# hku-mars/GS-SDF

Measured on NVIDIA H100. Metric: train_steps_per_s, higher is better.
Workload: dtype f32

## Files before the change

gs-sdf_b200/csrc/raster.cu:

```cuda
#include "common.cuh"
#include "conic.cuh"

namespace gssdf {

constexpr int kRasterThreads = 256;
constexpr int kRasterWarps = kRasterThreads / 32;
constexpr int kBatch = 128;
constexpr float kNearN = 0.05f, kFarN = 100.f;
constexpr float kAlphaThreshold = 1.f / 255.f;
constexpr int kRecF4 = 4;
constexpr int kRecBytes = kRecF4 * 16;

__global__ void __launch_bounds__(256)
pack_records_kernel(const gssdf_counts *counts, const float *__restrict__ ray_transforms,
                    const float *__restrict__ colors, const float *__restrict__ opacities,
                    const float *__restrict__ normals, float4 *__restrict__ rec, float4 *__restrict__ conic,
                    float *__restrict__ zero_a, int zero_a_stride, float extent) {
    const int nnz = counts->nnz;
    const int i = blockIdx.x * blockDim.x + threadIdx.x;
    if (i >= nnz) return;
    const float *M = ray_transforms + 9 * (int64_t)i;
    const float *c = colors + 3 * (int64_t)i;
    const float *n = normals + 3 * (int64_t)i;
    float4 *r = rec + kRecF4 * (int64_t)i;
    const float opac = opacities[i];
    r[0] = make_float4(M[0], M[1], M[2], M[3]);
    r[1] = make_float4(M[4], M[5], M[6], M[7]);
    r[2] = make_float4(M[8], opac, c[0], c[1]);
    r[3] = make_float4(c[2], n[0], n[1], n[2]);
    float q[6];
    uint32_t rect[2];
    splat_conic(M, opac, extent, q, rect);
    conic[kConicF4 * (int64_t)i] = make_float4(q[0], q[1], q[2], q[3]);
    conic[kConicF4 * (int64_t)i + 1] = make_float4(q[4], q[5], __uint_as_float(rect[0]), __uint_as_float(rect[1]));
    if (zero_a) {
        for (int k = 0; k < zero_a_stride; ++k) zero_a[(int64_t)i * zero_a_stride + k] = 0.f;
    }
}

__global__ void __launch_bounds__(256)
splat_conics_kernel(const gssdf_counts *counts, const float *__restrict__ ray_transforms, const float *__restrict__ opacities,
                    float4 *__restrict__ conic, float extent) {
    const int i = blockIdx.x * blockDim.x + threadIdx.x;
    if (i >= counts->nnz) return;
    float q[6];
    uint32_t rect[2];
    splat_conic(ray_transforms + 9 * (int64_t)i, opacities[i], extent, q, rect);
    conic[kConicF4 * (int64_t)i] = make_float4(q[0], q[1], q[2], q[3]);
    conic[kConicF4 * (int64_t)i + 1] = make_float4(q[4], q[5], __uint_as_float(rect[0]), __uint_as_float(rect[1]));
}

struct TileInfo {
    int cam, tile, rs, re;
    int tx, ty;
};

__device__ __forceinline__ TileInfo tile_info(int C, int tw, int th, const int32_t *offsets, const gssdf_counts *counts) {
    TileInfo t;
    const int n_tiles = tw * th;
    const int bin = blockIdx.x;
    t.cam = bin / n_tiles;
    t.tile = bin % n_tiles;
    t.ty = t.tile / tw;
    t.tx = t.tile % tw;
    const int n_isects = counts->n_isects;
    t.rs = min(offsets[bin], n_isects);
    t.re = (bin == C * n_tiles - 1) ? n_isects : min(offsets[bin + 1], n_isects);
    return t;
}

__device__ __forceinline__ void pixel_of_thread(int &lx, int &ly) {
    const int lane = threadIdx.x & 31, warp = threadIdx.x >> 5;
    lx = (warp & 1) * 8 + (lane & 7);
    ly = (warp >> 1) * 4 + (lane >> 3);
}

struct __align__(16) Stage {
    float4 rec[kBatch * kRecF4];
    int ids[kBatch];
    int meta[kBatch];
    float acc[kRasterWarps][kBatch];
};

__global__ void __launch_bounds__(kRasterThreads)
tile_cull_kernel(int C, int tw, int th, const int32_t *__restrict__ offsets, const gssdf_counts *counts,
                 const int32_t *__restrict__ flatten_ids, const float4 *__restrict__ conic, int2 *__restrict__ clist,
                 int32_t *__restrict__ ccount) {
    __shared__ int s_wc[kRasterThreads / 32];
    const TileInfo ti = tile_info(C, tw, th, offsets, counts);
    const float ox = ti.tx * kTile + 0.5f, oy = ti.ty * kTile + 0.5f;
    const int lane = threadIdx.x & 31, warp = threadIdx.x >> 5;
    int count = 0;
    for (int c0 = ti.rs; c0 < ti.re; c0 += kRasterThreads) {
        const int idx = c0 + threadIdx.x;
        int g = 0;
        unsigned mask = 0u;
        if (idx < ti.re) {
            g = flatten_ids[idx];
            mask = cull_mask(__ldg(conic + kConicF4 * (int64_t)g), __ldg(conic + kConicF4 * (int64_t)g + 1), ox, oy);
        }
        const unsigned bal = __ballot_sync(0xffffffffu, mask != 0u);
        if (lane == 0) s_wc[warp] = __popc(bal);
        __syncthreads();
        int before = 0, total = 0;
#pragma unroll
        for (int w = 0; w < kRasterThreads / 32; ++w) {
            const int c = s_wc[w];
            if (w < warp) before += c;
            total += c;
        }
        if (mask != 0u) clist[ti.rs + count + before + __popc(bal & ((1u << lane) - 1u))] = make_int2(g, ((idx - ti.rs) << 8) | (int)mask);
        count += total;
        __syncthreads();
    }
    if (threadIdx.x == 0) ccount[blockIdx.x] = count;
}

__device__ __forceinline__ void issue_batch(Stage &st, uint64_t *bar, const float4 *__restrict__ rec,
                                            const int2 *__restrict__ clist, int start, int n) {
    const int t = threadIdx.x;
    if (t < n) {
        const int2 e = clist[start + t];
        st.ids[t] = e.x;
        st.meta[t] = e.y;
#pragma unroll
        for (int w = 0; w < kRasterWarps; ++w) st.acc[w][t] = 0.f;
        bulk_g2s(&st.rec[t * kRecF4], rec + kRecF4 * (int64_t)e.x, kRecBytes, bar);
        mbar_arrive_expect_tx(bar, kRecBytes);
    } else {
        mbar_arrive(bar);
    }
}

template <bool DISTORT>
__global__ void __launch_bounds__(kRasterThreads)
raster2dgs_fwd_kernel(const gssdf_raster2dgs_fwd_args a, const float4 *__restrict__ rec, const int2 *__restrict__ clist,
                      const int32_t *__restrict__ ccount, int tw, int th) {
    extern __shared__ __align__(16) unsigned char s_raw_fwd[];
    Stage *s_stage = reinterpret_cast<Stage *>(s_raw_fwd);
    __shared__ __align__(8) uint64_t s_bar[2];
    const TileInfo ti = tile_info(a.C, tw, th, a.offsets, a.counts);
    const int W = a.image_width, H = a.image_height;
    int lx, ly;
    pixel_of_thread(lx, ly);
    const int i = ti.ty * kTile + ly, j = ti.tx * kTile + lx;
    const bool inside = i < H && j < W;
    const float px = (float)j + 0.5f, py = (float)i + 0.5f;
    const int64_t pix = ((int64_t)ti.cam * H + i) * W + j;
    const int lane = threadIdx.x & 31;

    if (threadIdx.x == 0) {
        mbar_init(&s_bar[0], kRasterThreads);
        mbar_init(&s_bar[1], kRasterThreads);
        fence_mbar_init();
    }
    __syncthreads();

    const int n_total = ccount[blockIdx.x];
    const int c_end = ti.rs + n_total;
    const int nb = (n_total + kBatch - 1) / kBatch;
    if (nb > 0) issue_batch(s_stage[0], &s_bar[0], rec, clist, ti.rs, min(kBatch, n_total));
    if (nb > 1) issue_batch(s_stage[1], &s_bar[1], rec, clist, ti.rs + kBatch, min(kBatch, n_total - kBatch));

    float T = 1.f;
    float pc0 = 0.f, pc1 = 0.f, pc2 = 0.f, pn0 = 0.f, pn1 = 0.f, pn2 = 0.f;
    float dout = 0.f, M1 = 0.f, M2 = 0.f, distort = 0.f, median_depth = 0.f;
    int cur_idx = 0, median_idx = 0;
    bool done = !inside;
    int waited = 0;

    for (int b = 0; b < nb; ++b) {
        Stage &st = s_stage[b & 1];
        mbar_wait(&s_bar[b & 1], (b >> 1) & 1);
        waited = b + 1;
        const int start = ti.rs + b * kBatch;
        const int bn = min(kBatch, c_end - start);
        const int warp_id = threadIdx.x >> 5;
        for (int t0 = 0; t0 < bn; t0 += 32) {
          if (__all_sync(0xffffffffu, done)) break;
          const int my_meta = (t0 + lane < bn) ? st.meta[t0 + lane] : 0;
          unsigned todo = __ballot_sync(0xffffffffu, (my_meta >> warp_id) & 1);
          while (todo) {
            const int src = __ffs(todo) - 1;
            const int t = t0 + src;
            todo &= todo - 1;
            if (__all_sync(0xffffffffu, done)) break;
            const int sorted_idx = ti.rs + (__shfl_sync(0xffffffffu, my_meta, src) >> 8);
            const float4 r0 = st.rec[t * kRecF4 + 0], r1 = st.rec[t * kRecF4 + 1], r2 = st.rec[t * kRecF4 + 2], r3 = st.rec[t * kRecF4 + 3];
            const float hux = px * r1.z - r0.x, huy = px * r1.w - r0.y, huz = px * r2.x - r0.z;
            const float hvx = py * r1.z - r0.w, hvy = py * r1.w - r1.x, hvz = py * r2.x - r1.y;
            const float rcx = huy * hvz - huz * hvy, rcy = huz * hvx - hux * hvz, rcz = hux * hvy - huy * hvx;
            bool ok = !done && rcz != 0.f;
            const float inv_rcz = __fdividef(1.f, rcz);
            const float sx = rcx * inv_rcz, sy = rcy * inv_rcz;
            const float sigma = 0.5f * (sx * sx + sy * sy);
            const float depth = sx * r1.z + sy * r1.w + r2.x;
            ok = ok && !(depth < kNearN);
            const float alpha = fminf(0.999f, r2.y * __expf(-sigma));
            ok = ok && !(sigma < 0.f || alpha < kAlphaThreshold);
            const float next_T = T * (1.f - alpha);
            if (ok && next_T <= 1e-4f) { done = true; ok = false; }
            float vis = 0.f;
            if (ok) {
                vis = alpha * T;
                pc0 += r2.z * vis; pc1 += r2.w * vis; pc2 += r3.x * vis;
                dout += depth * vis;
                pn0 += r3.y * vis; pn1 += r3.z * vis; pn2 += r3.w * vis;
                if (DISTORT) {
                    const float A = 1.f - T;
                    const float m = kFarN / (kFarN - kNearN) * (1.f - kNearN / depth);
                    distort += (m * m * A + M1 - 2.f * m * M2) * vis;
                    M1 += m * m * vis;
                    M2 += m * vis;
                }
                if (T > 0.5f) { median_depth = depth; median_idx = sorted_idx; }
                cur_idx = sorted_idx;
                T = next_T;
            }
            if (__any_sync(0xffffffffu, ok)) {
                const float v = warp_sum(vis);
                if (lane == 0) st.acc[warp_id][t] = v;
            }
          }
        }
        const int n_done = __syncthreads_count(done);
        if (threadIdx.x < bn) {
            float v = 0.f;
#pragma unroll
            for (int w = 0; w < kRasterWarps; ++w) v += st.acc[w][threadIdx.x];
            if (v != 0.f) atomicAdd(a.visibilities + st.ids[threadIdx.x], v);
        }
        if (n_done == kRasterThreads) break;
        __syncthreads();
        if (b + 2 < nb) {
            const int s2 = ti.rs + (b + 2) * kBatch;
            issue_batch(st, &s_bar[b & 1], rec, clist, s2, min(kBatch, c_end - s2));
        }
    }
    {
        const int issued = min(nb, waited + 1);
        for (int b = waited; b < issued; ++b) mbar_wait(&s_bar[b & 1], (b >> 1) & 1);
    }

    if (inside) {
        a.render_depths[pix] = dout;
        a.render_alphas[pix] = 1.f - T;
        if (DISTORT) reinterpret_cast<float2 *>(a.render_Ts)[pix] = make_float2(M1, M2);
        float b0 = 0.f, b1 = 0.f, b2 = 0.f;
        if (a.backgrounds) { b0 = a.backgrounds[3 * ti.cam]; b1 = a.backgrounds[3 * ti.cam + 1]; b2 = a.backgrounds[3 * ti.cam + 2]; }
        a.render_colors[3 * pix] = pc0 + T * b0;
        a.render_colors[3 * pix + 1] = pc1 + T * b1;
        a.render_colors[3 * pix + 2] = pc2 + T * b2;
        a.render_normals[3 * pix] = pn0;
        a.render_normals[3 * pix + 1] = pn1;
        a.render_normals[3 * pix + 2] = pn2;
        a.last_ids[pix] = cur_idx;
        if (DISTORT) a.render_distort[pix] = distort;
        a.render_median[pix] = median_depth;
        a.median_ids[pix] = median_idx;
    }
}

constexpr int kBwdThreads = 128;
constexpr int kBwdWarps = kBwdThreads / 32;
constexpr int kBwdBatch = 64;
constexpr int kBwdMinBlocks = 5;

template <bool ABS>
struct __align__(16) BwdStageT {
    float4 rec[kBwdBatch * kRecF4];
    float part[kBwdWarps * kBwdBatch * 16];
    float gabs[ABS ? kBwdWarps * 2 * kBwdBatch : 4];
    int ids[kBwdBatch];
    int meta[kBwdBatch];
};

template <bool ABS>
__device__ __forceinline__ void issue_batch_bwd(BwdStageT<ABS> &st, uint64_t *bar, const float4 *__restrict__ rec,
                                                const int2 *__restrict__ clist, int last, int n) {
    const int t = threadIdx.x;
    float4 *part4 = reinterpret_cast<float4 *>(st.part);
#pragma unroll
    for (int k = t; k < kBwdWarps * kBwdBatch * 4; k += kBwdThreads) part4[k] = make_float4(0.f, 0.f, 0.f, 0.f);
    if (ABS) {
#pragma unroll
        for (int k = t; k < kBwdWarps * 2 * kBwdBatch; k += kBwdThreads) st.gabs[k] = 0.f;
    }
    if (t < n) {
        const int2 e = clist[last - t];
        st.ids[t] = e.x;
        st.meta[t] = e.y;
        bulk_g2s(&st.rec[t * kRecF4], rec + kRecF4 * (int64_t)e.x, kRecBytes, bar);
        mbar_arrive_expect_tx(bar, kRecBytes);
    } else {
        mbar_arrive(bar);
    }
}

struct BwdPixel {
    float T;
    float bc0, bc1, bc2, bn0, bn1, bn2, bd;
    float vc0, vc1, vc2, vd, va, vn0, vn1, vn2, v_median;
    int bin_final, median_idx;
};

__device__ __forceinline__ void bwd_pixel_init(BwdPixel &P, const gssdf_raster2dgs_bwd_args &a, const TileInfo &ti, int lx, int ly) {
    const int W = a.image_width, H = a.image_height;
    const int i = ti.ty * kTile + ly, j = ti.tx * kTile + lx;
    const bool inside = i < H && j < W;
    const int64_t pix = inside ? ((int64_t)ti.cam * H + i) * W + j : 0;
    P.T = inside ? 1.f - a.render_alphas[pix] : 1.f;
    P.bc0 = P.bc1 = P.bc2 = P.bn0 = P.bn1 = P.bn2 = P.bd = 0.f;
    P.bin_final = inside ? a.last_ids[pix] : -1;
    P.median_idx = inside ? a.median_ids[pix] : -1;
    P.vc0 = P.vc1 = P.vc2 = P.vd = P.va = P.vn0 = P.vn1 = P.vn2 = P.v_median = 0.f;
    if (inside) {
        P.vc0 = a.v_render_colors[3 * pix]; P.vc1 = a.v_render_colors[3 * pix + 1]; P.vc2 = a.v_render_colors[3 * pix + 2];
        P.vd = a.v_render_depths[pix];
        P.va = a.v_render_alphas[pix];
        P.vn0 = a.v_render_normals[3 * pix]; P.vn1 = a.v_render_normals[3 * pix + 1]; P.vn2 = a.v_render_normals[3 * pix + 2];
        P.v_median = a.v_render_median[pix];
    }
    if (a.backgrounds)
        P.va -= a.backgrounds[3 * ti.cam] * P.vc0 + a.backgrounds[3 * ti.cam + 1] * P.vc1 + a.backgrounds[3 * ti.cam + 2] * P.vc2;
    P.va *= P.T;
}

__device__ __forceinline__ bool bwd_pixel_splat(BwdPixel &P, float px, float py, int idx, const float4 r0, const float4 r1, const float4 r2,
                                                const float4 r3, float g[16]) {
    const float hux = px * r1.z - r0.x, huy = px * r1.w - r0.y, huz = px * r2.x - r0.z;
    const float hvx = py * r1.z - r0.w, hvy = py * r1.w - r1.x, hvz = py * r2.x - r1.y;
    const float rcx = huy * hvz - huz * hvy, rcy = huz * hvx - hux * hvz, rcz = hux * hvy - huy * hvx;
    bool valid = idx <= P.bin_final && rcz != 0.f;
    const float inv_rcz = __fdividef(1.f, rcz);
    const float sx = rcx * inv_rcz, sy = rcy * inv_rcz;
    const float sigma = 0.5f * (sx * sx + sy * sy);
    const float depth = sx * r1.z + sy * r1.w + r2.x;
    valid = valid && !(depth < kNearN);
    const float opac = r2.y;
    const float vis = __expf(-sigma);
    const float alpha = fminf(0.999f, opac * vis);
    valid = valid && !(sigma < 0.f || alpha < kAlphaThreshold);
    if (valid) {
        float v_depth = (idx == P.median_idx) ? P.v_median : 0.f;
        const float ra = __fdividef(1.f, 1.f - alpha);
        P.T *= ra;
        const float T = P.T;
        const float fac = alpha * T;
        g[0] += fac * P.vc0; g[1] += fac * P.vc1; g[2] += fac * P.vc2;
        g[3] += fac * P.vn0; g[4] += fac * P.vn1; g[5] += fac * P.vn2;
        float v_alpha = (r2.z * T - P.bc0 * ra) * P.vc0 + (r2.w * T - P.bc1 * ra) * P.vc1 + (r3.x * T - P.bc2 * ra) * P.vc2;
        v_alpha += (r3.y * T - P.bn0 * ra) * P.vn0 + (r3.z * T - P.bn1 * ra) * P.vn1 + (r3.w * T - P.bn2 * ra) * P.vn2;
        v_alpha += ra * P.va;
        v_alpha += (depth * T - P.bd * ra) * P.vd;
        if (opac * vis <= 0.999f) {
            v_depth += fac * P.vd;
            const float v_G = opac * v_alpha;
            const float vsx = v_G * -vis * sx + v_depth * r1.z;
            const float vsy = v_G * -vis * sy + v_depth * r1.w;
            const float vsxz = vsx * inv_rcz, vsyz = vsy * inv_rcz;
            const float vrx = vsxz, vry = vsyz, vrz = -(vsxz * sx + vsyz * sy);
            const float vhux = hvy * vrz - hvz * vry, vhuy = hvz * vrx - hvx * vrz, vhuz = hvx * vry - hvy * vrx;
            const float vhvx = vry * huz - vrz * huy, vhvy = vrz * hux - vrx * huz, vhvz = vrx * huy - vry * hux;
            g[6] -= vhux; g[7] -= vhuy; g[8] -= vhuz;
            g[9] -= vhvx; g[10] -= vhvy; g[11] -= vhvz;
            g[12] += px * vhux + py * vhvx + v_depth * sx;
            g[13] += px * vhuy + py * vhvy + v_depth * sy;
            g[14] += px * vhuz + py * vhvz + v_depth;
            g[15] += vis * v_alpha;
        }
        P.bc0 += r2.z * fac; P.bc1 += r2.w * fac; P.bc2 += r3.x * fac;
        P.bd += depth * fac;
        P.bn0 += r3.y * fac; P.bn1 += r3.z * fac; P.bn2 += r3.w * fac;
    }
    return valid;
}

template <bool ABS>
__global__ void __launch_bounds__(kBwdThreads, kBwdMinBlocks)
raster2dgs_bwd_kernel(const gssdf_raster2dgs_bwd_args a, const float4 *__restrict__ rec, const int2 *__restrict__ clist,
                      const int32_t *__restrict__ ccount, float *__restrict__ vrec, int tw, int th) {
    using BwdStage = BwdStageT<ABS>;
    extern __shared__ __align__(16) unsigned char s_raw[];
    BwdStage *s_stage = reinterpret_cast<BwdStage *>(s_raw);
    __shared__ __align__(8) uint64_t s_bar[2];
    const TileInfo ti = tile_info(a.C, tw, th, a.offsets, a.counts);
    const int n_total = ccount[blockIdx.x];
    if (n_total <= 0) return;
    const int c_last = ti.rs + n_total - 1;
    const int lane = threadIdx.x & 31, warp = threadIdx.x >> 5;
    const int wb = (warp & 1) + 4 * (warp >> 1);
    const int lx = (warp & 1) * 8 + (lane & 7), ly = (warp >> 1) * 8 + (lane >> 3);
    const float px = (float)(ti.tx * kTile + lx) + 0.5f, py = (float)(ti.ty * kTile + ly) + 0.5f;

    if (threadIdx.x == 0) {
        mbar_init(&s_bar[0], kBwdThreads);
        mbar_init(&s_bar[1], kBwdThreads);
        fence_mbar_init();
    }
    __syncthreads();

    BwdPixel P0, P1;
    bwd_pixel_init(P0, a, ti, lx, ly);
    bwd_pixel_init(P1, a, ti, lx, ly + 4);
    const int warp_bin_final = warp_max_i(max(P0.bin_final, P1.bin_final));

    const int nb = (n_total + kBwdBatch - 1) / kBwdBatch;
    issue_batch_bwd(s_stage[0], &s_bar[0], rec, clist, c_last, min(kBwdBatch, n_total));
    if (nb > 1) issue_batch_bwd(s_stage[1], &s_bar[1], rec, clist, c_last - kBwdBatch, min(kBwdBatch, n_total - kBwdBatch));

    for (int b = 0; b < nb; ++b) {
        BwdStage &st = s_stage[b & 1];
        mbar_wait(&s_bar[b & 1], (b >> 1) & 1);
        const int last = c_last - b * kBwdBatch;
        const int bn = min(kBwdBatch, last - ti.rs + 1);
        float *part = st.part + warp * kBwdBatch * 16;
        for (int t0 = 0; t0 < bn; t0 += 32) {
          const int my_meta = (t0 + lane < bn) ? st.meta[t0 + lane] : 0;
          unsigned todo = __ballot_sync(0xffffffffu, ((my_meta >> wb) & 5) && (ti.rs + (my_meta >> 8) <= warp_bin_final));
          while (todo) {
            const int src = __ffs(todo) - 1;
            const int t = t0 + src;
            todo &= todo - 1;
            const int m = __shfl_sync(0xffffffffu, my_meta, src);
            const int idx = ti.rs + (m >> 8);
            const float4 r0 = st.rec[t * kRecF4 + 0], r1 = st.rec[t * kRecF4 + 1], r2 = st.rec[t * kRecF4 + 2], r3 = st.rec[t * kRecF4 + 3];
            float g[16];
#pragma unroll
            for (int k = 0; k < 16; ++k) g[k] = 0.f;
            bool any = false;
            if ((m >> wb) & 1) any = bwd_pixel_splat(P0, px, py, idx, r0, r1, r2, r3, g);
            if ((m >> (wb + 2)) & 1) any |= bwd_pixel_splat(P1, px, py + 4.f, idx, r0, r1, r2, r3, g);
            if (!__any_sync(0xffffffffu, any)) continue;

            float h8[8], h4[4], h2[2], h1;
            const bool b4 = lane & 16, b3 = lane & 8, b2 = lane & 4, b1 = lane & 2;
#pragma unroll
            for (int k = 0; k < 8; ++k) {
                const float send = b4 ? g[k] : g[k + 8], keep = b4 ? g[k + 8] : g[k];
                h8[k] = keep + __shfl_xor_sync(0xffffffffu, send, 16);
            }
#pragma unroll
            for (int k = 0; k < 4; ++k) {
                const float send = b3 ? h8[k] : h8[k + 4], keep = b3 ? h8[k + 4] : h8[k];
                h4[k] = keep + __shfl_xor_sync(0xffffffffu, send, 8);
            }
#pragma unroll
            for (int k = 0; k < 2; ++k) {
                const float send = b2 ? h4[k] : h4[k + 2], keep = b2 ? h4[k + 2] : h4[k];
                h2[k] = keep + __shfl_xor_sync(0xffffffffu, send, 4);
            }
            {
                const float send = b1 ? h2[0] : h2[1], keep = b1 ? h2[1] : h2[0];
                h1 = keep + __shfl_xor_sync(0xffffffffu, send, 2);
            }
            h1 += __shfl_xor_sync(0xffffffffu, h1, 1);
            const int comp = lane >> 1;
            if ((lane & 1) == 0) part[t * 16 + comp] = h1;
            if (ABS) {
                if (lane == 16) st.gabs[(2 * warp) * kBwdBatch + t] = fabsf(h1 * r2.x);
                if (lane == 22) st.gabs[(2 * warp + 1) * kBwdBatch + t] = fabsf(h1 * r2.x);
            }
          }
        }
        __syncthreads();
        const float4 *part4 = reinterpret_cast<const float4 *>(st.part);
        for (int e = threadIdx.x; e < bn * 4; e += kBwdThreads) {
            float4 v = part4[e];
#pragma unroll
            for (int w = 1; w < kBwdWarps; ++w) {
                const float4 p = part4[w * kBwdBatch * 4 + e];
                v.x += p.x; v.y += p.y; v.z += p.z; v.w += p.w;
            }
            if (v.x != 0.f || v.y != 0.f || v.z != 0.f || v.w != 0.f)
                atomicAdd(reinterpret_cast<float4 *>(vrec) + 4 * (int64_t)st.ids[e >> 2] + (e & 3), v);
        }
        if (ABS) {
            for (int e = threadIdx.x; e < bn * 2; e += kBwdThreads) {
                const int t = e >> 1, k = e & 1;
                float v = 0.f;
#pragma unroll
                for (int w = 0; w < kBwdWarps; ++w) v += st.gabs[(2 * w + k) * kBwdBatch + t];
                if (v != 0.f) atomicAdd(a.v_means2d_abs + 2 * (int64_t)st.ids[t] + k, v);
            }
        }
        __syncthreads();
        if (b + 2 < nb) {
            const int l2 = c_last - (b + 2) * kBwdBatch;
            issue_batch_bwd(st, &s_bar[b & 1], rec, clist, l2, min(kBwdBatch, l2 - ti.rs + 1));
        }
    }
}

__global__ void __launch_bounds__(256)
raster_bwd_finalize_kernel(const gssdf_raster2dgs_bwd_args a, const float4 *__restrict__ vrec) {
    const int nnz = a.counts->nnz;
    const int i = blockIdx.x * blockDim.x + threadIdx.x;
    if (i >= nnz) return;
    const float4 g0 = vrec[4 * (int64_t)i], g1 = vrec[4 * (int64_t)i + 1], g2 = vrec[4 * (int64_t)i + 2], g3 = vrec[4 * (int64_t)i + 3];
    float *vc = a.v_colors + 3 * (int64_t)i;
    vc[0] = g0.x; vc[1] = g0.y; vc[2] = g0.z;
    float *vn = a.v_normals + 3 * (int64_t)i;
    vn[0] = g0.w; vn[1] = g1.x; vn[2] = g1.y;
    float *vm = a.v_ray_transforms + 9 * (int64_t)i;
    vm[0] = g1.z; vm[1] = g1.w; vm[2] = g2.x;
    vm[3] = g2.y; vm[4] = g2.z; vm[5] = g2.w;
    vm[6] = g3.x; vm[7] = g3.y; vm[8] = g3.z;
    a.v_opacities[i] = g3.w;
    if (a.v_means2d) { a.v_means2d[2 * (int64_t)i] = 0.f; a.v_means2d[2 * (int64_t)i + 1] = 0.f; }
    if (a.v_densify) {
        const float mz = a.ray_transforms[9 * (int64_t)i + 8];
        a.v_densify[2 * (int64_t)i] = g2.x * mz;
        a.v_densify[2 * (int64_t)i + 1] = g2.w * mz;
    }
}

__device__ __forceinline__ void cam_rot(const float *viewmats, int cam, float R[9]) {
    const float *v = viewmats + 16 * cam;
#pragma unroll
    for (int r = 0; r < 3; ++r)
#pragma unroll
        for (int c = 0; c < 3; ++c) R[r * 3 + c] = v[r * 4 + c];
}

__global__ void __launch_bounds__(256) render_post_fwd_kernel(const gssdf_render_post_fwd_args a) {
    const int64_t P = (int64_t)a.image_width * a.image_height;
    const int64_t p = (int64_t)blockIdx.x * blockDim.x + threadIdx.x;
    if (p >= P * a.C) return;
    const int cam = (int)(p / P);
    float R[9];
    cam_rot(a.viewmats, cam, R);
    const float al = a.render_alphas[p], d = a.render_depths[p];
    float ed = d / al;
    if (isnan(ed)) ed = 0.f;
    else if (isinf(ed)) ed = ed > 0 ? 3.402823466e38f : -3.402823466e38f;
    reinterpret_cast<float4 *>(a.out_colors)[p] =
        make_float4(a.render_colors[3 * p], a.render_colors[3 * p + 1], a.render_colors[3 * p + 2], ed);
    const float n0 = a.render_normals[3 * p], n1 = a.render_normals[3 * p + 1], n2 = a.render_normals[3 * p + 2];
#pragma unroll
    for (int c = 0; c < 3; ++c) a.out_normals[3 * p + c] = n0 * R[c] + n1 * R[3 + c] + n2 * R[6 + c];
}

__global__ void __launch_bounds__(256) render_post_bwd_kernel(const gssdf_render_post_bwd_args a) {
    const int64_t P = (int64_t)a.image_width * a.image_height;
    const int64_t p = (int64_t)blockIdx.x * blockDim.x + threadIdx.x;
    if (p >= P * a.C) return;
    const int cam = (int)(p / P);
    float R[9];
    cam_rot(a.viewmats, cam, R);
    const float4 vo = reinterpret_cast<const float4 *>(a.v_out_colors)[p];
    a.v_render_colors[3 * p] = vo.x; a.v_render_colors[3 * p + 1] = vo.y; a.v_render_colors[3 * p + 2] = vo.z;
    const float al = a.render_alphas[p], d = a.render_depths[p];
    const float ed = d / al;
    float vdep = 0.f, val = a.v_alphas_in ? a.v_alphas_in[p] : 0.f;
    if (!(isnan(ed) || isinf(ed))) {
        vdep = vo.w / al;
        val += -vo.w * d / (al * al);
    }
    a.v_render_depths[p] = vdep;
    a.v_render_alphas[p] = val;
    const float g0 = a.v_out_normals[3 * p], g1 = a.v_out_normals[3 * p + 1], g2 = a.v_out_normals[3 * p + 2];
#pragma unroll
    for (int r = 0; r < 3; ++r) a.v_render_normals[3 * p + r] = g0 * R[r * 3] + g1 * R[r * 3 + 1] + g2 * R[r * 3 + 2];
}

__global__ void __launch_bounds__(256) l1_loss_kernel(const gssdf_l1_loss_args a, int64_t n_pix) {
    const int64_t p = (int64_t)blockIdx.x * blockDim.x + threadIdx.x;
    float part = 0.f;
    if (p < n_pix) {
        const float4 o = reinterpret_cast<const float4 *>(a.out_colors)[p];
        const float4 g = reinterpret_cast<const float4 *>(a.gt)[p];
        const float sr = a.w_rgb / (3.f * (float)n_pix), sd = a.w_depth / (float)n_pix;
        const float d0 = o.x - g.x, d1 = o.y - g.y, d2 = o.z - g.z, d3 = o.w - g.w;
        part = sr * (fabsf(d0) + fabsf(d1) + fabsf(d2)) + sd * fabsf(d3);
        auto sgn = [](float x) { return x > 0.f ? 1.f : (x < 0.f ? -1.f : 0.f); };
        reinterpret_cast<float4 *>(a.v_out_colors)[p] = make_float4(sr * sgn(d0), sr * sgn(d1), sr * sgn(d2), sd * sgn(d3));
    }
    part = warp_sum(part);
    __shared__ float s_part[8];
    if ((threadIdx.x & 31) == 0) s_part[threadIdx.x >> 5] = part;
    __syncthreads();
    if (threadIdx.x == 0) {
        float s = 0.f;
        for (int w = 0; w < 8; ++w) s += s_part[w];
        atomicAdd(a.loss_out, s);
    }
}

}

using namespace gssdf;

extern "C" int gssdf_l1_loss(const gssdf_l1_loss_args *a, gssdf_stream_t stream) {
    GSSDF_REQUIRE(a != nullptr, GSSDF_EINVAL, "l1_loss: null args");
    GSSDF_REQUIRE(a->C > 0 && a->image_width > 0 && a->image_height > 0, GSSDF_EINVAL, "l1_loss: bad image size");
    GSSDF_REQUIRE(a->out_colors && a->gt && a->loss_out && a->v_out_colors, GSSDF_EINVAL, "l1_loss: null pointer");
    const int64_t n = (int64_t)a->C * a->image_width * a->image_height;
    l1_loss_kernel<<<cdiv(n, 256), 256, 0, (cudaStream_t)stream>>>(*a, n);
    GSSDF_LAUNCH_OK("l1_loss_kernel");
    return GSSDF_OK;
}

struct RasterWs {
    float4 *rec;
    float4 *conic;
    int2 *clist;
    int32_t *ccount;
    float4 *vrec;
    size_t fwd_bytes, bwd_bytes;
};

static RasterWs carve_ws(void *base, int C, int W, int H, int cap, int64_t isect_cap) {
    const size_t n = (size_t)(cap > 0 ? cap : 1), I = (size_t)(isect_cap > 0 ? isect_cap : 1);
    const size_t tiles = (size_t)(C > 0 ? C : 1) * cdiv(W > 0 ? W : 1, kTile) * cdiv(H > 0 ? H : 1, kTile);
    char *p = reinterpret_cast<char *>(base);
    RasterWs w;
    size_t off = 0;
    w.rec = reinterpret_cast<float4 *>(p + off); off += align_up(n * kRecBytes, 256);
    w.conic = reinterpret_cast<float4 *>(p + off); off += align_up(n * kConicF4 * 16, 256);
    w.clist = reinterpret_cast<int2 *>(p + off); off += align_up(I * sizeof(int2), 256);
    w.ccount = reinterpret_cast<int32_t *>(p + off); off += align_up(tiles * sizeof(int32_t), 256);
    w.fwd_bytes = off;
    w.vrec = reinterpret_cast<float4 *>(p + off); off += align_up(n * 64, 256);
    w.bwd_bytes = off;
    return w;
}

extern "C" size_t gssdf_raster2dgs_workspace_bytes(int32_t C, int32_t W, int32_t H, int32_t cap, int64_t isect_cap) {
    return carve_ws(nullptr, C, W, H, cap, isect_cap).fwd_bytes;
}
extern "C" size_t gssdf_raster2dgs_bwd_workspace_bytes(int32_t C, int32_t W, int32_t H, int32_t cap, int64_t isect_cap) {
    return carve_ws(nullptr, C, W, H, cap, isect_cap).bwd_bytes;
}

static int check_raster_common(const char *who, int C, int W, int H, int tile_size, int channels) {
    GSSDF_REQUIRE(C > 0 && W > 0 && H > 0, GSSDF_EINVAL, "%s: C, width, height must be positive", who);
    GSSDF_REQUIRE(tile_size == kTile, GSSDF_EUNSUPPORTED, "%s: tile_size %d unsupported (GS-SDF renders with 16)", who, tile_size);
    GSSDF_REQUIRE(channels == 3, channels <= 0 || channels > 512 ? GSSDF_EINVAL : GSSDF_EUNSUPPORTED,
                  "%s: Unsupported number of color channels: %d", who, channels);
    return GSSDF_OK;
}

extern "C" int gssdf_splat_conics(const gssdf_splat_conics_args *a, gssdf_stream_t stream) {
    GSSDF_REQUIRE(a != nullptr, GSSDF_EINVAL, "splat_conics: null args");
    GSSDF_REQUIRE(a->cap >= 0 && a->image_width > 0 && a->image_height > 0, GSSDF_EINVAL, "splat_conics: bad sizes");
    if (a->cap == 0) return GSSDF_OK;
    GSSDF_REQUIRE(a->counts && a->ray_transforms && a->opacities && a->conics, GSSDF_EINVAL, "splat_conics: null pointer");
    GSSDF_REQUIRE(((uintptr_t)a->conics & 15) == 0, GSSDF_EINVAL, "splat_conics: conics must be 16-byte aligned");
    splat_conics_kernel<<<cdiv(a->cap, 256), 256, 0, (cudaStream_t)stream>>>(a->counts, a->ray_transforms, a->opacities,
                                                                            reinterpret_cast<float4 *>(a->conics),
                                                                            (float)max(a->image_width, a->image_height));
    GSSDF_LAUNCH_OK("splat_conics_kernel");
    return GSSDF_OK;
}

static int pack_and_cull(const char *who, const RasterWs &w, const gssdf_counts *counts, int C, int W, int H, int cap,
                         const float *ray_transforms, const float *colors, const float *opacities, const float *normals,
                         const int32_t *offsets, const int32_t *flatten_ids, float *zero_a, int zero_stride, cudaStream_t st) {
    const int tw = cdiv(W, kTile), th = cdiv(H, kTile);
    if (cap > 0) {
        pack_records_kernel<<<cdiv(cap, 256), 256, 0, st>>>(counts, ray_transforms, colors, opacities, normals, w.rec, w.conic, zero_a,
                                                           zero_stride, (float)max(W, H));
        GSSDF_LAUNCH_OK("pack_records_kernel");
    }
    tile_cull_kernel<<<C * tw * th, kRasterThreads, 0, st>>>(C, tw, th, offsets, counts, flatten_ids, w.conic, w.clist, w.ccount);
    GSSDF_LAUNCH_OK("tile_cull_kernel");
    (void)who;
    return GSSDF_OK;
}

extern "C" int gssdf_raster2dgs_fwd(const gssdf_raster2dgs_fwd_args *a, gssdf_stream_t stream) {
    GSSDF_REQUIRE(a != nullptr, GSSDF_EINVAL, "raster2dgs_fwd: null args");
    int rc = check_raster_common("raster2dgs_fwd", a->C, a->image_width, a->image_height, a->tile_size, a->channels);
    if (rc) return rc;
    GSSDF_REQUIRE(a->counts && a->offsets && a->render_colors && a->render_depths && a->render_alphas && a->render_normals &&
                      a->render_median && a->last_ids && a->median_ids && (a->render_distort != nullptr) == (a->render_Ts != nullptr),
                  GSSDF_EINVAL, "raster2dgs_fwd: null output / counts / offsets");
    GSSDF_REQUIRE(a->cap == 0 || (a->ray_transforms && a->colors && a->opacities && a->normals && a->flatten_ids && a->visibilities),
                  GSSDF_EINVAL, "raster2dgs_fwd: null splat input");
    GSSDF_REQUIRE(a->isect_cap >= 0, GSSDF_EINVAL, "raster2dgs_fwd: negative isect_cap");
    GSSDF_REQUIRE(a->workspace && a->workspace_bytes >= gssdf_raster2dgs_workspace_bytes(a->C, a->image_width, a->image_height, a->cap,
                                                                                         a->isect_cap),
                  GSSDF_ENOMEM, "raster2dgs_fwd: workspace too small");
    cudaStream_t st = (cudaStream_t)stream;
    const int tw = cdiv(a->image_width, kTile), th = cdiv(a->image_height, kTile);
    const RasterWs w = carve_ws(a->workspace, a->C, a->image_width, a->image_height, a->cap, a->isect_cap);
    rc = pack_and_cull("raster2dgs_fwd", w, a->counts, a->C, a->image_width, a->image_height, a->cap, a->ray_transforms, a->colors,
                       a->opacities, a->normals, a->offsets, a->flatten_ids, a->visibilities, 1, st);
    if (rc) return rc;
    GSSDF_CUDA_OK(cudaFuncSetAttribute(raster2dgs_fwd_kernel<true>, cudaFuncAttributeMaxDynamicSharedMemorySize, (int)(2 * sizeof(Stage))));
    GSSDF_CUDA_OK(cudaFuncSetAttribute(raster2dgs_fwd_kernel<false>, cudaFuncAttributeMaxDynamicSharedMemorySize, (int)(2 * sizeof(Stage))));
    if (a->prof_start) GSSDF_CUDA_OK(cudaEventRecord((cudaEvent_t)a->prof_start, st));
    if (a->render_distort)
        raster2dgs_fwd_kernel<true><<<a->C * tw * th, kRasterThreads, 2 * sizeof(Stage), st>>>(*a, w.rec, w.clist, w.ccount, tw, th);
    else
        raster2dgs_fwd_kernel<false><<<a->C * tw * th, kRasterThreads, 2 * sizeof(Stage), st>>>(*a, w.rec, w.clist, w.ccount, tw, th);
    GSSDF_LAUNCH_OK("raster2dgs_fwd_kernel");
    if (a->prof_stop) GSSDF_CUDA_OK(cudaEventRecord((cudaEvent_t)a->prof_stop, st));
    return GSSDF_OK;
}

extern "C" int gssdf_raster2dgs_bwd(const gssdf_raster2dgs_bwd_args *a, gssdf_stream_t stream) {
    GSSDF_REQUIRE(a != nullptr, GSSDF_EINVAL, "raster2dgs_bwd: null args");
    int rc = check_raster_common("raster2dgs_bwd", a->C, a->image_width, a->image_height, a->tile_size, a->channels);
    if (rc) return rc;
    GSSDF_REQUIRE(a->v_render_distort == nullptr, GSSDF_EUNSUPPORTED,
                  "raster2dgs_bwd: distortion-loss cotangent is outside the GS-SDF path (distloss=false)");
    if (a->cap == 0) return GSSDF_OK;
    GSSDF_REQUIRE(a->counts && a->offsets && a->flatten_ids && a->ray_transforms && a->colors && a->opacities && a->normals &&
                      a->render_alphas && a->last_ids && a->median_ids && a->v_render_colors && a->v_render_depths &&
                      a->v_render_alphas && a->v_render_normals && a->v_render_median,
                  GSSDF_EINVAL, "raster2dgs_bwd: null input");
    GSSDF_REQUIRE(a->v_ray_transforms && a->v_colors && a->v_opacities && a->v_normals, GSSDF_EINVAL, "raster2dgs_bwd: null output");
    GSSDF_REQUIRE(a->isect_cap >= 0, GSSDF_EINVAL, "raster2dgs_bwd: negative isect_cap");
    GSSDF_REQUIRE(a->workspace && a->workspace_bytes >= gssdf_raster2dgs_bwd_workspace_bytes(a->C, a->image_width, a->image_height,
                                                                                             a->cap, a->isect_cap),
                  GSSDF_ENOMEM, "raster2dgs_bwd: workspace too small");
    cudaStream_t st = (cudaStream_t)stream;
    const int tw = cdiv(a->image_width, kTile), th = cdiv(a->image_height, kTile);
    const RasterWs w = carve_ws(a->workspace, a->C, a->image_width, a->image_height, a->cap, a->isect_cap);
    if (!a->reuse_fwd) {
        rc = pack_and_cull("raster2dgs_bwd", w, a->counts, a->C, a->image_width, a->image_height, a->cap, a->ray_transforms, a->colors,
                           a->opacities, a->normals, a->offsets, a->flatten_ids, nullptr, 0, st);
        if (rc) return rc;
    }
    GSSDF_CUDA_OK(cudaMemsetAsync(w.vrec, 0, (size_t)a->cap * 64, st));
    if (a->v_means2d_abs) GSSDF_CUDA_OK(cudaMemsetAsync(a->v_means2d_abs, 0, (size_t)a->cap * 2 * sizeof(float), st));
    if (a->prof_start) GSSDF_CUDA_OK(cudaEventRecord((cudaEvent_t)a->prof_start, st));
    auto launch = [&](auto kern, size_t smem) -> int {
        GSSDF_CUDA_OK(cudaFuncSetAttribute(kern, cudaFuncAttributeMaxDynamicSharedMemorySize, (int)smem));
        kern<<<a->C * tw * th, kBwdThreads, smem, st>>>(*a, w.rec, w.clist, w.ccount, reinterpret_cast<float *>(w.vrec), tw, th);
        return GSSDF_OK;
    };
    rc = a->v_means2d_abs ? launch(raster2dgs_bwd_kernel<true>, 2 * sizeof(BwdStageT<true>))
                          : launch(raster2dgs_bwd_kernel<false>, 2 * sizeof(BwdStageT<false>));
    if (rc) return rc;
    GSSDF_LAUNCH_OK("raster2dgs_bwd_kernel");
    if (a->prof_stop) GSSDF_CUDA_OK(cudaEventRecord((cudaEvent_t)a->prof_stop, st));
    raster_bwd_finalize_kernel<<<cdiv(a->cap, 256), 256, 0, st>>>(*a, w.vrec);
    GSSDF_LAUNCH_OK("raster_bwd_finalize_kernel");
    return GSSDF_OK;
}

extern "C" int gssdf_render_post_fwd(const gssdf_render_post_fwd_args *a, gssdf_stream_t stream) {
    GSSDF_REQUIRE(a != nullptr, GSSDF_EINVAL, "render_post_fwd: null args");
    GSSDF_REQUIRE(a->C > 0 && a->image_width > 0 && a->image_height > 0, GSSDF_EINVAL, "render_post_fwd: bad image size");
    GSSDF_REQUIRE(a->viewmats && a->render_colors && a->render_depths && a->render_alphas && a->render_normals && a->out_colors &&
                      a->out_normals,
                  GSSDF_EINVAL, "render_post_fwd: null pointer");
    const int64_t n = (int64_t)a->C * a->image_width * a->image_height;
    render_post_fwd_kernel<<<cdiv(n, 256), 256, 0, (cudaStream_t)stream>>>(*a);
    GSSDF_LAUNCH_OK("render_post_fwd_kernel");
    return GSSDF_OK;
}

extern "C" int gssdf_render_post_bwd(const gssdf_render_post_bwd_args *a, gssdf_stream_t stream) {
    GSSDF_REQUIRE(a != nullptr, GSSDF_EINVAL, "render_post_bwd: null args");
    GSSDF_REQUIRE(a->C > 0 && a->image_width > 0 && a->image_height > 0, GSSDF_EINVAL, "render_post_bwd: bad image size");
    GSSDF_REQUIRE(a->viewmats && a->render_depths && a->render_alphas && a->v_out_colors && a->v_out_normals && a->v_render_colors &&
                      a->v_render_depths && a->v_render_alphas && a->v_render_normals,
                  GSSDF_EINVAL, "render_post_bwd: null pointer");
    const int64_t n = (int64_t)a->C * a->image_width * a->image_height;
    render_post_bwd_kernel<<<cdiv(n, 256), 256, 0, (cudaStream_t)stream>>>(*a);
    GSSDF_LAUNCH_OK("render_post_bwd_kernel");
    return GSSDF_OK;
}
```

Baseline: 192.7.

## Have each forward raster thread shade two pixels with half the threads per tile

The forward rasterizer now launches 128 threads per 16x16 tile, and each thread composites two pixels four rows apart. The shared-memory splat record is loaded once and reused for both pixels, and per-warp ballots skip splats whose cull-mask bits miss both halves. The change also swaps __expf for a direct ex2.approx, sets min-blocks launch bounds, and refreshes warp liveness only when a pixel saturates. The cost is higher register pressure, with two sets of accumulators per thread, plus more divergent branching in the inner loop.

```diff
diff --git a/gs-sdf_b200/csrc/raster.cu b/gs-sdf_b200/csrc/raster.cu
--- a/gs-sdf_b200/csrc/raster.cu
+++ b/gs-sdf_b200/csrc/raster.cu
@@ -4,8 +4,6 @@
 namespace gssdf {
 
 constexpr int kRasterThreads = 256;
-constexpr int kRasterWarps = kRasterThreads / 32;
-constexpr int kBatch = 128;
 constexpr float kNearN = 0.05f, kFarN = 100.f;
 constexpr float kAlphaThreshold = 1.f / 255.f;
 constexpr int kRecF4 = 4;
@@ -69,17 +67,17 @@
     return t;
 }
 
-__device__ __forceinline__ void pixel_of_thread(int &lx, int &ly) {
-    const int lane = threadIdx.x & 31, warp = threadIdx.x >> 5;
-    lx = (warp & 1) * 8 + (lane & 7);
-    ly = (warp >> 1) * 4 + (lane >> 3);
-}
+constexpr int kFwdThreads = 128;
+constexpr int kFwdWarps = kFwdThreads / 32;
+constexpr int kBatch = 128;
+constexpr int kFwdMinBlocks = 8;
+constexpr int kFwdMinBlocksDistort = 6;
 
 struct __align__(16) Stage {
     float4 rec[kBatch * kRecF4];
     int ids[kBatch];
     int meta[kBatch];
-    float acc[kRasterWarps][kBatch];
+    float acc[kFwdWarps][kBatch];
 };
 
 __global__ void __launch_bounds__(kRasterThreads)
@@ -124,7 +122,7 @@
         st.ids[t] = e.x;
         st.meta[t] = e.y;
 #pragma unroll
-        for (int w = 0; w < kRasterWarps; ++w) st.acc[w][t] = 0.f;
+        for (int w = 0; w < kFwdWarps; ++w) st.acc[w][t] = 0.f;
         bulk_g2s(&st.rec[t * kRecF4], rec + kRecF4 * (int64_t)e.x, kRecBytes, bar);
         mbar_arrive_expect_tx(bar, kRecBytes);
     } else {
@@ -132,8 +130,95 @@
     }
 }
 
+static_assert(kBatch <= kFwdThreads, "issue_batch gathers one record per thread");
+
+__device__ __forceinline__ float exp_neg_half(float rho2) {
+    float y;
+    asm("ex2.approx.ftz.f32 %0, %1;" : "=f"(y) : "f"(rho2 * (-0.5f * 1.4426950408889634f)));
+    return y;
+}
+
+struct FwdPixel {
+    float T;
+    float pc0, pc1, pc2, pn0, pn1, pn2, dout, median_depth;
+    float M1, M2, distort;
+    int cur_idx, median_idx;
+    bool done;
+};
+
+struct FwdHit {
+    float alpha, depth;
+    bool ok;
+};
+
+__device__ __forceinline__ FwdHit fwd_pixel_test(const FwdPixel &P, float px, float py, const float4 r0, const float4 r1, const float4 r2) {
+    const float hux = px * r1.z - r0.x, huy = px * r1.w - r0.y, huz = px * r2.x - r0.z;
+    const float hvx = py * r1.z - r0.w, hvy = py * r1.w - r1.x, hvz = py * r2.x - r1.y;
+    const float rcx = huy * hvz - huz * hvy, rcy = huz * hvx - hux * hvz, rcz = hux * hvy - huy * hvx;
+    FwdHit h;
+    h.ok = !P.done && rcz != 0.f;
+    const float inv_rcz = __fdividef(1.f, rcz);
+    const float sx = rcx * inv_rcz, sy = rcy * inv_rcz;
+    const float rho2 = sx * sx + sy * sy;
+    h.depth = sx * r1.z + sy * r1.w + r2.x;
+    h.ok = h.ok && !(h.depth < kNearN);
+    h.alpha = fminf(0.999f, r2.y * exp_neg_half(rho2));
+    h.ok = h.ok && !(h.alpha < kAlphaThreshold);
+    return h;
+}
+
 template <bool DISTORT>
-__global__ void __launch_bounds__(kRasterThreads)
+__device__ __forceinline__ float fwd_pixel_composite(FwdPixel &P, const FwdHit h, int sorted_idx, const float4 r2, const float4 *r, bool &stop) {
+    const float alpha = h.alpha, depth = h.depth;
+    bool ok = h.ok;
+    const float next_T = P.T * (1.f - alpha);
+    if (ok && next_T <= 1e-4f) { P.done = true; stop = true; ok = false; }
+    float vis = 0.f;
+    if (ok) {
+        const float4 r3 = r[3];
+        vis = alpha * P.T;
+        P.pc0 += r2.z * vis; P.pc1 += r2.w * vis; P.pc2 += r3.x * vis;
+        P.dout += depth * vis;
+        P.pn0 += r3.y * vis; P.pn1 += r3.z * vis; P.pn2 += r3.w * vis;
+        if (DISTORT) {
+            const float A = 1.f - P.T;
+            const float m = kFarN / (kFarN - kNearN) * (1.f - kNearN / depth);
+            P.distort += (m * m * A + P.M1 - 2.f * m * P.M2) * vis;
+            P.M1 += m * m * vis;
+            P.M2 += m * vis;
+        }
+        if (P.T > 0.5f) { P.median_depth = depth; P.median_idx = sorted_idx; }
+        P.cur_idx = sorted_idx;
+        P.T = next_T;
+    }
+    return vis;
+}
+
+template <bool DISTORT>
+__device__ __forceinline__ void fwd_pixel_store(const FwdPixel &P, const gssdf_raster2dgs_fwd_args &a, const TileInfo &ti, int lx, int ly) {
+    const int W = a.image_width, H = a.image_height;
+    const int i = ti.ty * kTile + ly, j = ti.tx * kTile + lx;
+    if (i >= H || j >= W) return;
+    const int64_t pix = ((int64_t)ti.cam * H + i) * W + j;
+    a.render_depths[pix] = P.dout;
+    a.render_alphas[pix] = 1.f - P.T;
+    if (DISTORT) reinterpret_cast<float2 *>(a.render_Ts)[pix] = make_float2(P.M1, P.M2);
+    float b0 = 0.f, b1 = 0.f, b2 = 0.f;
+    if (a.backgrounds) { b0 = a.backgrounds[3 * ti.cam]; b1 = a.backgrounds[3 * ti.cam + 1]; b2 = a.backgrounds[3 * ti.cam + 2]; }
+    a.render_colors[3 * pix] = P.pc0 + P.T * b0;
+    a.render_colors[3 * pix + 1] = P.pc1 + P.T * b1;
+    a.render_colors[3 * pix + 2] = P.pc2 + P.T * b2;
+    a.render_normals[3 * pix] = P.pn0;
+    a.render_normals[3 * pix + 1] = P.pn1;
+    a.render_normals[3 * pix + 2] = P.pn2;
+    a.last_ids[pix] = P.cur_idx;
+    if (DISTORT) a.render_distort[pix] = P.distort;
+    a.render_median[pix] = P.median_depth;
+    a.median_ids[pix] = P.median_idx;
+}
+
+template <bool DISTORT>
+__global__ void __launch_bounds__(kFwdThreads, DISTORT ? kFwdMinBlocksDistort : kFwdMinBlocks)
 raster2dgs_fwd_kernel(const gssdf_raster2dgs_fwd_args a, const float4 *__restrict__ rec, const int2 *__restrict__ clist,
                       const int32_t *__restrict__ ccount, int tw, int th) {
     extern __shared__ __align__(16) unsigned char s_raw_fwd[];
@@ -141,17 +226,15 @@
     __shared__ __align__(8) uint64_t s_bar[2];
     const TileInfo ti = tile_info(a.C, tw, th, a.offsets, a.counts);
     const int W = a.image_width, H = a.image_height;
-    int lx, ly;
-    pixel_of_thread(lx, ly);
+    const int lane = threadIdx.x & 31, warp = threadIdx.x >> 5;
+    const int wb = (warp & 1) + 4 * (warp >> 1);
+    const int lx = (warp & 1) * 8 + (lane & 7), ly = (warp >> 1) * 8 + (lane >> 3);
     const int i = ti.ty * kTile + ly, j = ti.tx * kTile + lx;
-    const bool inside = i < H && j < W;
     const float px = (float)j + 0.5f, py = (float)i + 0.5f;
-    const int64_t pix = ((int64_t)ti.cam * H + i) * W + j;
-    const int lane = threadIdx.x & 31;
 
     if (threadIdx.x == 0) {
-        mbar_init(&s_bar[0], kRasterThreads);
-        mbar_init(&s_bar[1], kRasterThreads);
+        mbar_init(&s_bar[0], kFwdThreads);
+        mbar_init(&s_bar[1], kFwdThreads);
         fence_mbar_init();
     }
     __syncthreads();
@@ -162,11 +245,16 @@
     if (nb > 0) issue_batch(s_stage[0], &s_bar[0], rec, clist, ti.rs, min(kBatch, n_total));
     if (nb > 1) issue_batch(s_stage[1], &s_bar[1], rec, clist, ti.rs + kBatch, min(kBatch, n_total - kBatch));
 
-    float T = 1.f;
-    float pc0 = 0.f, pc1 = 0.f, pc2 = 0.f, pn0 = 0.f, pn1 = 0.f, pn2 = 0.f;
-    float dout = 0.f, M1 = 0.f, M2 = 0.f, distort = 0.f, median_depth = 0.f;
-    int cur_idx = 0, median_idx = 0;
-    bool done = !inside;
+    FwdPixel P0, P1;
+    P0.T = P1.T = 1.f;
+    P0.pc0 = P0.pc1 = P0.pc2 = P0.pn0 = P0.pn1 = P0.pn2 = P0.dout = P0.median_depth = P0.M1 = P0.M2 = P0.distort = 0.f;
+    P1.pc0 = P1.pc1 = P1.pc2 = P1.pn0 = P1.pn1 = P1.pn2 = P1.dout = P1.median_depth = P1.M1 = P1.M2 = P1.distort = 0.f;
+    P0.cur_idx = P0.median_idx = P1.cur_idx = P1.median_idx = 0;
+    P0.done = !(i < H && j < W);
+    P1.done = !(i + 4 < H && j < W);
+    auto live_halves = [&]() { return (__all_sync(0xffffffffu, P0.done) ? 0 : 1) | (__all_sync(0xffffffffu, P1.done) ? 0 : 4); };
+    int live = live_halves();
+    const float py1 = py + 4.f;
     int waited = 0;
 
     for (int b = 0; b < nb; ++b) {
@@ -175,62 +263,51 @@
         waited = b + 1;
         const int start = ti.rs + b * kBatch;
         const int bn = min(kBatch, c_end - start);
-        const int warp_id = threadIdx.x >> 5;
         for (int t0 = 0; t0 < bn; t0 += 32) {
-          if (__all_sync(0xffffffffu, done)) break;
+          if (!live) break;
           const int my_meta = (t0 + lane < bn) ? st.meta[t0 + lane] : 0;
-          unsigned todo = __ballot_sync(0xffffffffu, (my_meta >> warp_id) & 1);
+          unsigned todo0 = __ballot_sync(0xffffffffu, (my_meta >> wb) & live & 1);
+          unsigned todo1 = __ballot_sync(0xffffffffu, (my_meta >> wb) & live & 4);
+          unsigned todo = todo0 | todo1;
           while (todo) {
             const int src = __ffs(todo) - 1;
             const int t = t0 + src;
             todo &= todo - 1;
-            if (__all_sync(0xffffffffu, done)) break;
             const int sorted_idx = ti.rs + (__shfl_sync(0xffffffffu, my_meta, src) >> 8);
-            const float4 r0 = st.rec[t * kRecF4 + 0], r1 = st.rec[t * kRecF4 + 1], r2 = st.rec[t * kRecF4 + 2], r3 = st.rec[t * kRecF4 + 3];
-            const float hux = px * r1.z - r0.x, huy = px * r1.w - r0.y, huz = px * r2.x - r0.z;
-            const float hvx = py * r1.z - r0.w, hvy = py * r1.w - r1.x, hvz = py * r2.x - r1.y;
-            const float rcx = huy * hvz - huz * hvy, rcy = huz * hvx - hux * hvz, rcz = hux * hvy - huy * hvx;
-            bool ok = !done && rcz != 0.f;
-            const float inv_rcz = __fdividef(1.f, rcz);
-            const float sx = rcx * inv_rcz, sy = rcy * inv_rcz;
-            const float sigma = 0.5f * (sx * sx + sy * sy);
-            const float depth = sx * r1.z + sy * r1.w + r2.x;
-            ok = ok && !(depth < kNearN);
-            const float alpha = fminf(0.999f, r2.y * __expf(-sigma));
-            ok = ok && !(sigma < 0.f || alpha < kAlphaThreshold);
-            const float next_T = T * (1.f - alpha);
-            if (ok && next_T <= 1e-4f) { done = true; ok = false; }
+            const float4 *r = &st.rec[t * kRecF4];
+            const float4 r0 = r[0], r1 = r[1], r2 = r[2];
             float vis = 0.f;
-            if (ok) {
-                vis = alpha * T;
-                pc0 += r2.z * vis; pc1 += r2.w * vis; pc2 += r3.x * vis;
-                dout += depth * vis;
-                pn0 += r3.y * vis; pn1 += r3.z * vis; pn2 += r3.w * vis;
-                if (DISTORT) {
-                    const float A = 1.f - T;
-                    const float m = kFarN / (kFarN - kNearN) * (1.f - kNearN / depth);
-                    distort += (m * m * A + M1 - 2.f * m * M2) * vis;
-                    M1 += m * m * vis;
-                    M2 += m * vis;
-                }
-                if (T > 0.5f) { median_depth = depth; median_idx = sorted_idx; }
-                cur_idx = sorted_idx;
-                T = next_T;
-            }
-            if (__any_sync(0xffffffffu, ok)) {
+            bool stop = false;
+            const bool u0 = (todo0 >> src) & 1, u1 = (todo1 >> src) & 1;
+            if (u0 && u1) {
+                const FwdHit h0 = fwd_pixel_test(P0, px, py, r0, r1, r2), h1 = fwd_pixel_test(P1, px, py1, r0, r1, r2);
+                vis = fwd_pixel_composite<DISTORT>(P0, h0, sorted_idx, r2, r, stop);
+                vis += fwd_pixel_composite<DISTORT>(P1, h1, sorted_idx, r2, r, stop);
+            } else if (u0) {
+                vis = fwd_pixel_composite<DISTORT>(P0, fwd_pixel_test(P0, px, py, r0, r1, r2), sorted_idx, r2, r, stop);
+            } else {
+                vis = fwd_pixel_composite<DISTORT>(P1, fwd_pixel_test(P1, px, py1, r0, r1, r2), sorted_idx, r2, r, stop);
+            }
+            if (__any_sync(0xffffffffu, vis != 0.f)) {
                 const float v = warp_sum(vis);
-                if (lane == 0) st.acc[warp_id][t] = v;
+                if (lane == 0) st.acc[warp][t] = v;
+            }
+            if (__any_sync(0xffffffffu, stop)) {
+                live = live_halves();
+                if (!(live & 1)) todo0 = 0u;
+                if (!(live & 4)) todo1 = 0u;
+                todo &= todo0 | todo1;
             }
           }
         }
-        const int n_done = __syncthreads_count(done);
+        const int n_done = __syncthreads_count(P0.done && P1.done);
         if (threadIdx.x < bn) {
             float v = 0.f;
 #pragma unroll
-            for (int w = 0; w < kRasterWarps; ++w) v += st.acc[w][threadIdx.x];
+            for (int w = 0; w < kFwdWarps; ++w) v += st.acc[w][threadIdx.x];
             if (v != 0.f) atomicAdd(a.visibilities + st.ids[threadIdx.x], v);
         }
-        if (n_done == kRasterThreads) break;
+        if (n_done == kFwdThreads) break;
         __syncthreads();
         if (b + 2 < nb) {
             const int s2 = ti.rs + (b + 2) * kBatch;
@@ -242,23 +319,8 @@
         for (int b = waited; b < issued; ++b) mbar_wait(&s_bar[b & 1], (b >> 1) & 1);
     }
 
-    if (inside) {
-        a.render_depths[pix] = dout;
-        a.render_alphas[pix] = 1.f - T;
-        if (DISTORT) reinterpret_cast<float2 *>(a.render_Ts)[pix] = make_float2(M1, M2);
-        float b0 = 0.f, b1 = 0.f, b2 = 0.f;
-        if (a.backgrounds) { b0 = a.backgrounds[3 * ti.cam]; b1 = a.backgrounds[3 * ti.cam + 1]; b2 = a.backgrounds[3 * ti.cam + 2]; }
-        a.render_colors[3 * pix] = pc0 + T * b0;
-        a.render_colors[3 * pix + 1] = pc1 + T * b1;
-        a.render_colors[3 * pix + 2] = pc2 + T * b2;
-        a.render_normals[3 * pix] = pn0;
-        a.render_normals[3 * pix + 1] = pn1;
-        a.render_normals[3 * pix + 2] = pn2;
-        a.last_ids[pix] = cur_idx;
-        if (DISTORT) a.render_distort[pix] = distort;
-        a.render_median[pix] = median_depth;
-        a.median_ids[pix] = median_idx;
-    }
+    fwd_pixel_store<DISTORT>(P0, a, ti, lx, ly);
+    fwd_pixel_store<DISTORT>(P1, a, ti, lx, ly + 4);
 }
 
 constexpr int kBwdThreads = 128;
@@ -692,9 +754,9 @@
     GSSDF_CUDA_OK(cudaFuncSetAttribute(raster2dgs_fwd_kernel<false>, cudaFuncAttributeMaxDynamicSharedMemorySize, (int)(2 * sizeof(Stage))));
     if (a->prof_start) GSSDF_CUDA_OK(cudaEventRecord((cudaEvent_t)a->prof_start, st));
     if (a->render_distort)
-        raster2dgs_fwd_kernel<true><<<a->C * tw * th, kRasterThreads, 2 * sizeof(Stage), st>>>(*a, w.rec, w.clist, w.ccount, tw, th);
+        raster2dgs_fwd_kernel<true><<<a->C * tw * th, kFwdThreads, 2 * sizeof(Stage), st>>>(*a, w.rec, w.clist, w.ccount, tw, th);
     else
-        raster2dgs_fwd_kernel<false><<<a->C * tw * th, kRasterThreads, 2 * sizeof(Stage), st>>>(*a, w.rec, w.clist, w.ccount, tw, th);
+        raster2dgs_fwd_kernel<false><<<a->C * tw * th, kFwdThreads, 2 * sizeof(Stage), st>>>(*a, w.rec, w.clist, w.ccount, tw, th);
     GSSDF_LAUNCH_OK("raster2dgs_fwd_kernel");
     if (a->prof_stop) GSSDF_CUDA_OK(cudaEventRecord((cudaEvent_t)a->prof_stop, st));
     return GSSDF_OK;
```

Result: faster. 194.7, median of 6 (+1.0%).
